# linchaobao/EPPM

Measured on AMD Instinct MI355X. Metric: Mflow-vectors/sec, higher is better.
Workload: dtype f32; 1 GPU; single 1024x436 Sintel-shape synthetic pair per step, full 3-level pyramid, patch_r=9, default defs.h parameters; 1 rank(s), independent pairs; inputs: RGBA planes resident in HBM before the timed region; outputs: interleaved float2 flow left in HBM (the PCIe-inclusive window of the reference API -- host RGB in, host u/v out -- is `host_boundary`, with --full); inputs=device-resident RGBA, outputs=device-resident float2 flow, pairs_in_flight_per_gpu=24, pairs_per_launch=8, contexts_in_flight=3, width=1024, height=436

## Files before the change

eppm_amd/_lib.py:

```python
import ctypes as C
import os

from .build import lib_path


class EppmError(RuntimeError):
    pass


class CParams(C.Structure):
    _fields_ = [("patch_r", C.c_int), ("num_iter", C.c_int), ("search_range", C.c_int), ("num_guess", C.c_int),
                ("seg_len", C.c_int), ("wmf_iters", C.c_int), ("seed", C.c_ulonglong), ("propagation", C.c_int),
                ("levels", C.c_int)]


class CTrackParams(C.Structure):
    _fields_ = [("spacing", C.c_int), ("min_eig", C.c_int64), ("fb_alpha", C.c_float), ("fb_beta", C.c_float), ("mb_alpha", C.c_float),
                ("mb_beta", C.c_float), ("capacity", C.c_int)]


class CTFilterParams(C.Structure):
    _fields_ = [("thresh", C.c_float), ("n_max", C.c_int)]


# ... 42 lines not shown
    "eppm_device_synchronize", "eppm_device_mem_info", "eppm_device_pci_bus_id", "eppm_bind_thread_to_device", "eppm_release_cached_memory", "eppm_set_launcher_stream", "eppm_set_launcher_params", "eppm_launcher_status",
    "baoCudaPatchMatchMultiscalePrepare", "baoCudaCensusTransform", "baoCudaPatchMatch", "baoCudaLeftRightCheck",
    "baoCudaOutlierRemoval", "baoCudaWeightedMedianFilter", "baoCudaFillHole", "baoCudaNNF2Flow", "baoCudaBLF_C2F",
    "baoCudaBLFCostFilterRefine", "baoCudaFlowSmoothing", "eppm_flow_to_color", "eppm_compute_color",
    "eppm_pm_rng_create", "eppm_pm_rng_reset", "eppm_pm_rng_destroy", "eppm_pm_rng_block_states", "eppm_pm_gen_rand_field",
    "eppm_pm_cost_field", "eppm_pm_seg_propagate", "eppm_pm_jump_propagate", "eppm_pm_parallel_propagate", "eppm_pm_random_search", "eppm_gauss_filter_rgba", "eppm_resize_rgba",
    "eppm_resize_flow",
    "eppm_host_register", "eppm_host_unregister", "eppm_host_is_registered", "eppm_host_alloc", "eppm_host_free",
    "eppm_compute_begin_into", "eppm_batch_compute_begin_into",
    "eppm_load_ppm", "eppm_ppm_size", "eppm_save_flo", "eppm_load_flo", "eppm_flo_size", "eppm_flow_error",
    "eppm_flow_error_border", "eppm_flow_error_percentage", "eppm_flow_cutoff", "eppm_flow_to_color_host",
    "eppm_compute_bidirectional", "eppm_compute_bidirectional_device", "eppm_batch_compute_bidirectional", "eppm_set_occlusion_params",
    "eppm_fb_occlusion", "eppm_fb_occlusion_host",
    "eppm_interpolate", "eppm_interpolate_device", "eppm_batch_interpolate", "eppm_interpolate_frames", "eppm_interpolate_host",
    "eppm_track_default_params", "eppm_track_capacity", "eppm_tracker_create", "eppm_tracker_destroy", "eppm_track_step",
    "eppm_track_step_frames", "eppm_tracker_get", "eppm_tracker_get_ended", "eppm_tracker_set", "eppm_track_step_host", "eppm_track_seeds_host",
    "eppm_push_image", "eppm_push_image_device", "eppm_set_temporal", "eppm_temporal_reset", "eppm_temporal_valid", "eppm_temporal_prior_host",
    "eppm_temporal_prior",
    "eppm_batch_set_temporal", "eppm_batch_push_images", "eppm_batch_push_images_device", "eppm_batch_temporal_valid", "eppm_batch_temporal_reset",
    "eppm_temporal_prior_batch",
    "eppm_set_stop_level", "eppm_stop_level", "eppm_flow_upsample",
    "eppm_tfilter_default_params", "eppm_tfilter_create", "eppm_tfilter_create_size", "eppm_tfilter_destroy", "eppm_tfilter_reset", "eppm_tfilter_step",
    "eppm_tfilter_step_frames", "eppm_tfilter_get", "eppm_tfilter_get_device", "eppm_tfilter_get_state", "eppm_tfilter_set_state",
    "eppm_tfilter_seed_host", "eppm_tfilter_step_host",
    "eppm_stab_default_params", "eppm_stab_create", "eppm_stab_create_size", "eppm_stab_destroy", "eppm_stab_reset", "eppm_stab_step",
    "eppm_stab_step_frames", "eppm_stab_get", "eppm_stab_get_device", "eppm_stab_get_mask", "eppm_stab_get_model", "eppm_stab_get_path",
    "eppm_stab_set_path", "eppm_gmotion_fit_host", "eppm_stab_update_host", "eppm_stab_warp_host",
    "eppm_cutdet_default_params", "eppm_cutdet_create", "eppm_cutdet_create_size", "eppm_cutdet_destroy", "eppm_cutdet_step",
    "eppm_cutdet_step_frames", "eppm_cutdet_get", "eppm_cutdet_cuts", "eppm_cutdet_host",
]


TEST_SYMBOLS = ["eppm_test_set_option", "eppm_probe_c2f_window", "eppm_probe_dispatch", "eppm_probe_fast_exp", "eppm_probe_div_const", "eppm_probe_delta_table",
                "eppm_probe_unpack_texel", "eppm_probe_pm_parity", "eppm_probe_ctx_rng_states"]

_variant = None


def select_library(variant):
    global _variant
    if _lib is not None and variant != _variant:
        raise EppmError("select_library: a library is loaded already")
    _variant = variant


def lib():
    global _lib
    if _lib is None:
        path = lib_path(_variant)
        if not os.path.exists(path):
            raise EppmError(f"{path} is missing: run eppm_amd.build() (hipcc --offload-arch=gfx950); there is no CPU fallback")
        L = C.CDLL(path)
        L.eppm_last_error.restype = C.c_char_p
        L.eppm_version.restype = C.c_char_p
        _lib = L
    return _lib


def check(status, what=""):
    if status != 0:
        raise EppmError(f"{what}: status {status}: {lib().eppm_last_error().decode()}")


def check_launcher(what=""):
    check(lib().eppm_launcher_status(), what)


def probe_dispatch(stage, *args, nout=1):
    a = (C.c_int * len(args))(*[int(v) for v in args])
    out = (C.c_int * nout)()
    check(lib().eppm_probe_dispatch(stage.encode(), a, len(args), out, nout), f"eppm_probe_dispatch {stage}")
    return tuple(out)
```

eppm_amd/csrc/c2f_device.cuh:

```cuda
#pragma once
#include "eppm_device.cuh"

#ifndef EPPM_C2F_UNROLL
#define EPPM_C2F_UNROLL 2
#endif
#ifndef EPPM_C2F_WAVES
#define EPPM_C2F_WAVES 4
#endif
#ifndef EPPM_C2F_WAVES_MIN
#define EPPM_C2F_WAVES_MIN 2
#endif
#define EPPM_C2F_OCC __attribute__((amdgpu_waves_per_eu(EPPM_C2F_WAVES_MIN, EPPM_C2F_WAVES)))
#ifndef EPPM_C2F_WIN_H
#ifdef EPPM_TOL
#define EPPM_C2F_WIN_H 50
#else
#define EPPM_C2F_WIN_H 48
#endif
#endif
#ifndef EPPM_C2F_PASS2
#define EPPM_C2F_PASS2 1
#endif
#ifndef EPPM_C2F_WIN_WAVES
#define EPPM_C2F_WIN_WAVES 4
// ... 31 lines not shown
    return pk[idx];
}

__device__ __forceinline__ bool c2f_unknown(float fvx, float fvy) { return fvx > kUnknownFlowThresh || fvy > kUnknownFlowThresh; }
__device__ __forceinline__ int c2f_centre(float f, int x) { return (int)(int16_t)(f2short(f) + x); }
__device__ __forceinline__ void c2f_store_flow(float* flow, int idx, int fx, int fy)
{
    flow[idx * 2] = (float)fx;
    flow[idx * 2 + 1] = (float)fy;
}
__device__ __forceinline__ float c2f_min(float a, float b) { return (a < b) ? a : b; }
__device__ __forceinline__ float c2f_min4(float c1, float c2, float c3, float c4) { return c2f_min(c1, c2f_min(c2, c2f_min(c3, c4))); }
template <class F>
__device__ __forceinline__ void c2f_select_best(float* flow, int x, int y, int ccx, int ccy, int w, int h, F cost_of)
{
    int bx = ccx, by = ccy;
    float min_cost = 999999;
#pragma unroll
    for (int m = 0; m < 3; m++) {
        const int cx = (int)(int16_t)(ccx + m - 1);
        if (cx < 0 || cx >= w) continue;
#pragma unroll
        for (int n = 0; n < 3; n++) {
            const int cy = (int)(int16_t)(ccy + n - 1);
            if (cy < 0 || cy >= h) continue;
            const float cv = cost_of(m, n);
            if (cv < min_cost) { min_cost = cv; bx = cx; by = cy; }
        }
    }
    flow[(y * w + x) * 2] = (float)(bx - x);
    flow[(y * w + x) * 2 + 1] = (float)(by - y);
}

template <int SPLIT>
__device__ __forceinline__ bool c2f_tile_origin(const Planes& P, int& x0, int& y0, int& part)
{
    const int tiles_x = (P.w + kBlock - 1) / kBlock, tiles = tiles_x * ((P.h + kBlock - 1) / kBlock);
    const int per_xcd = (tiles + 7) / 8;
    const int slot = SPLIT ? (blockIdx.x >> 3) / SPLIT : (blockIdx.x >> 3);
    part = SPLIT ? (blockIdx.x >> 3) % SPLIT : -1;
    const int tile = (blockIdx.x & 7) * per_xcd + slot;
    if (slot >= per_xcd || tile >= tiles) return false;
    x0 = (tile % tiles_x) * kBlock; y0 = (tile / tiles_x) * kBlock;
    return true;
}

template <int R> struct C2fSrcTile { static constexpr int TWU = kBlock + 2 * R, TW = (TWU + 15) / 16 * 16; };
struct C2fOff { int dx16, up; };

template <int R>
struct C2fTables {
    static constexpr int S = R + 1;
    C2fOff off[3][S * S];
    int rowdy[3][S];
};

constexpr int cfloor(float v) { const int t = (int)v; return ((float)t > v) ? t - 1 : t; }
template <int R>
constexpr C2fTables<R> make_c2f_tables()
{
    constexpr int S = R + 1;
    constexpr float kc[3][4] = {
        {0.177f, -0.011f, -0.003f, 0.301f},
        {0.125f, -0.357f, 0.009f, 0.308f},
        {0.205f, 0.370f, 0.011f, 0.296f},
    };
    C2fTables<R> T{};
    for (int p = 0; p < 3; p++)
        for (int ii = 0; ii < S; ii++) {
            const int i = 2 * ii - R;
            int dy[S] = {};
            int lo = 1 << 30;
            for (int jj = 0; jj < S; jj++) {
                const int j = 2 * jj - R;
                const float fx = (float)(j)*kc[p][0] + (float)(i)*kc[p][1];
// ... 159 lines not shown
```

eppm_amd/csrc/context.h:

```cpp
#pragma once

#include <algorithm>

#include "api_internal.h"

struct StageEv { const char* name; hipEvent_t a, b; };

struct eppm_ctx {
    int device = 0;
    hipStream_t stream = nullptr;
    bool own_stream = false;
    int opt_sweep_spec = -1, opt_no_split = 0;
    eppm_params prm;
    int h = 0, w = 0, nl = 0;
    int stop_level = 0;
    int npairs = 1, n_active = 1;
    char* slab = nullptr;
    size_t stride = 0;
    int H[eppm::kMaxLevels], W[eppm::kMaxLevels];
    size_t ipitch[eppm::kMaxLevels], cpitch[eppm::kMaxLevels];
    uint32_t *raw1 = nullptr, *raw2 = nullptr;
    size_t raw_pitch = 0;
    uint32_t *img1[eppm::kMaxLevels] = {}, *img2[eppm::kMaxLevels] = {}, *tmpu[eppm::kMaxLevels] = {};
    uint8_t *cen1[eppm::kMaxLevels] = {}, *cen2[eppm::kMaxLevels] = {};
    void *pk1[eppm::kMaxLevels] = {}, *pk2[eppm::kMaxLevels] = {};
    uint32_t *pc1[eppm::kMaxLevels] = {}, *pc2[eppm::kMaxLevels] = {};
    uint32_t *pp1 = nullptr, *pp2 = nullptr;
    int pp_pitch = 0, pp_pad = 0;
    int16_t *nnf1 = nullptr, *nnf2 = nullptr, *nnf_tmp = nullptr, *nnf_tmp2 = nullptr;
    float *cost1 = nullptr, *cost2 = nullptr;
    float *spec1 = nullptr, *spec2 = nullptr;
    int32_t *scand1 = nullptr, *scand2 = nullptr;
    uint32_t *wl1 = nullptr, *wl2 = nullptr;
    int16_t *seed1 = nullptr, *seed2 = nullptr;
    uint32_t* wmf_ws = nullptr;
    bool flow_pending = false;
    float *flow[eppm::kMaxLevels] = {}, *flow_tmp[eppm::kMaxLevels] = {};
    float* c2f_cost9[eppm::kMaxLevels] = {};
    float *lut_pm = nullptr, *lut_wmf = nullptr, *lut_blf = nullptr;
    eppm_pm_rng* rng = nullptr;
    float* d_uv = nullptr;
    uint32_t* d_color = nullptr;
    uint32_t* h_color = nullptr;
    uint8_t* d_rgb = nullptr;
    size_t slab_bytes = 0, h_rgb_bytes = 0, h_flow_bytes = 0;
    uint8_t* h_rgb[2] = {nullptr, nullptr};
    hipEvent_t ev_rgb[2] = {nullptr, nullptr};
    hipEvent_t ev_h2d = nullptr;
    int rgb_cur = 0;
    float* h_flow = nullptr;
    std::vector<float*> out_u, out_v;
    eppm::HostHold out_hold;
    bool have_images = false, have_flow = false;
    char* bwd = nullptr;
    size_t bwd_stride = 0, bwd_bytes = 0, h_bwd_bytes = 0;
    float* bflow[eppm::kMaxLevels] = {};
    float* d_buv = nullptr;
    uint8_t *occ1 = nullptr, *occ2 = nullptr;
    uint8_t* h_bwd = nullptr;
    float occ_alpha = 0.01f, occ_beta = 0.5f;
    bool have_bwd = false;
    bool bwd_images = false;
    char* itp = nullptr;
    size_t itp_bytes = 0, itp_plane = 0, h_itp_bytes = 0;
    uint64_t* itp_keys = nullptr;
    int32_t *itp_fill1 = nullptr, *itp_fill2 = nullptr;
    uint8_t* itp_rgb = nullptr;
    uint8_t* h_itp = nullptr;
    bool temporal = false;
    std::vector<uint8_t> tmp_snap;
    std::vector<uint8_t> tmp_valid;
    std::vector<uint8_t> tmp_seeded;
    std::vector<uint8_t> tmp_cut;
    char* tmp = nullptr;
    size_t tmp_bytes = 0, tmp_stride = 0;
    int16_t *prev_fwd = nullptr, *prev_bwd = nullptr, *prior1 = nullptr, *prior2 = nullptr, *nnf_init1 = nullptr, *nnf_init2 = nullptr;
    float *cost_init1 = nullptr, *cost_init2 = nullptr;
    int32_t* tmp_keys = nullptr;
    void tmp_drop() { std::fill(tmp_valid.begin(), tmp_valid.end(), 0); std::fill(tmp_snap.begin(), tmp_snap.end(), 0); std::fill(tmp_cut.begin(), tmp_cut.end(), 0); }
    int timing = 0;
    std::vector<StageEv> ev;
    std::vector<StageEv> ev_prep;
    std::vector<hipEvent_t> ev_pool;
    eppm::Batch bt() const { return eppm::Batch{n_active, stride}; }
    template <class T> T* of_pair(T* p, int k) const { return (T*)((char*)p + (size_t)k * stride); }
    template <class T> T* of_bwd_pair(T* p, int k) const { return (T*)((char*)p + (size_t)k * bwd_stride); }
// ... 85 lines not shown
```

eppm_amd/csrc/ctx_compute.cpp:

```cpp
#include "context.h"
#include "temporal.h"

using namespace eppm;

static int tmp_alloc(eppm_ctx* c)
{
    if (c->tmp) return EPPM_OK;
    const int L = c->nl - 1;
    const size_t n2 = (size_t)c->W[L] * c->H[L];
    Carve cv;
    for (int16_t** p : {&c->prev_fwd, &c->prev_bwd, &c->prior1, &c->prior2, &c->nnf_init1, &c->nnf_init2}) cv.plane(p, n2 * 4);
    for (float** p : {&c->cost_init1, &c->cost_init2}) cv.plane(p, n2 * 4);
    cv.plane(&c->tmp_keys, n2 * 4 * 2);
    c->tmp_stride = cv.off;
    CHK(cv.alloc(&c->tmp, &c->tmp_bytes, c->tmp_stride * c->npairs, c->device, "temporal planes"));
    for (int k = 0; k < c->npairs; k++) launch_temporal_keys_init((int32_t*)((char*)c->tmp_keys + (size_t)k * c->tmp_stride), (int)(2 * n2), c->stream);
    HIPCHK(hipGetLastError());
    return EPPM_OK;
}

static int set_temporal(eppm_ctx* c, int on)
{
    c->temporal = on != 0;
    if (!on) c->tmp_drop();
// ... 68 lines not shown
static int branch_c2f(eppm_ctx* c, Branch& d, int (*keep)(eppm_ctx*, int, float*))
{
    hipStream_t s = c->stream;
    const Batch bt = c->bt();
    const int L = c->nl - 1;
    auto blf = [&](float* dst, const float* src, int l) { launch_flow_blf(dst, src, d.guide[l], (int)(c->ipitch[l] / 4), c->W[l], c->H[l], c->W[l], c->lut_blf, s, bt); };
    const int stop = c->stop_level;
    float* r = d.a[L];
    for (int l = L - 1; l >= 0; l--) {
        if (l < stop) {
            stage_begin(c, c->ev, level_stage.s[kStageJbu][d.bwd][l]);
            float* out = (r == d.b[l]) ? d.a[l] : d.b[l];
            launch_flow_jbu(out, r, d.guide[l], (int)(c->ipitch[l] / 4), c->W[l], c->H[l], c->W[l + 1], c->H[l + 1], c->lut_blf, s, bt);
            r = out;
            CHK(keep(c, l, r));
            stage_end(c, c->ev);
            continue;
        }
        stage_begin(c, c->ev, level_stage.s[kStageUp][d.bwd][l]);
        launch_resize_flow(d.a[l], c->H[l], c->W[l], r, c->H[l + 1], c->W[l + 1], 2.0f, 2.0f, s, bt);
        stage_end(c, c->ev);
        stage_begin(c, c->ev, level_stage.s[kStageRefine][d.bwd][l], d.dominant);
        launch_c2f_refine(planes(c, l, d.swap), d.a[l], c->lut_pm, c->prm.patch_r, c->c2f_cost9[l], s, bt, c->opt_no_split != 0);
        stage_end(c, c->ev, d.dominant);
        stage_begin(c, c->ev, level_stage.s[kStageBlf][d.bwd][l]);
        blf(d.b[l], d.a[l], l);
        r = d.b[l];
        if (l > 0) CHK(keep(c, l, r));
        stage_end(c, c->ev);
    }
    if (stop > 0) return EPPM_OK;
    stage_begin(c, c->ev, d.bwd ? "flow_blf_bwd_final" : "flow_blf_final");
    float* out = (r == d.b[0]) ? d.a[0] : d.b[0];
    blf(out, r, 0);
    CHK(keep(c, 0, out));
    stage_end(c, c->ev);
    return EPPM_OK;
}

static int keep_fwd(eppm_ctx* c, int l, float* r)
{
    if (r != c->flow[l]) std::swap(c->flow[l], c->flow_tmp[l]);
    return EPPM_OK;
}

static int compute_all(eppm_ctx* c)
{
    if (!c->have_images) return set_err(EPPM_ERR_STATE, "eppm_compute: no images set");
    HIPCHK(hipSetDevice(c->device));
    c->have_bwd = false;
    hipStream_t s = c->stream;
    const Batch bt = c->bt();
    const int L = c->nl - 1, lw = c->W[L], lh = c->H[L];

    const bool tmode = c->temporal;
    bool seeded = false;
    std::fill(c->tmp_seeded.begin(), c->tmp_seeded.end(), 0);
    if (tmode) {
        CHK(tmp_alloc(c));
        TemporalArgs a{};
        for (int k = 0; k < bt.n; k++)
            if (c->tmp_valid[k]) { a.armed[k >> 5] |= 1u << (k & 31); seeded = true; }
        if (seeded) {
            a.prev[0] = c->prev_fwd; a.prior[0] = c->prior1; a.keys[0] = c->tmp_keys; a.step[0] = 1;
            a.prev[1] = c->prev_bwd; a.prior[1] = c->prior2; a.keys[1] = c->tmp_keys + (size_t)lw * lh; a.step[1] = -1;
            a.w = lw; a.h = lh; a.ndir = 2; a.nslots = bt.n; a.stride = c->tmp_stride;
            stage_begin(c, c->ev, "temporal_advect");
// ... 70 lines not shown
        HIPCHK(hipMemcpyAsync(c->of_bwd_pair(c->bflow[l], k), c->of_pair(src, k), bytes, hipMemcpyDeviceToDevice, c->stream));
    return EPPM_OK;
}

static int backward_all(eppm_ctx* c)
{
    const int L = c->nl - 1;
    Branch d{c->nnf2, c->nnf_tmp2, c->cost2, c->img2, true, true, false, nullptr};
    for (int l = 0; l <= L; l++) { d.a[l] = c->flow_tmp[l]; d.b[l] = c->d_uv; }
    stage_begin(c, c->ev, "l2_post_bwd");
    branch_nnf2flow(c, d);
    if (L > 0) CHK(keep_bwd(c, L, d.a[L]));
    stage_end(c, c->ev);
    CHK(branch_c2f(c, d, keep_bwd));

    stage_begin(c, c->ev, "fb_occlusion");
    launch_fb_occlusion(c->occ1, c->occ2, c->flow[0], c->stride, c->bflow[0], c->bwd_stride, c->h, c->w, c->occ_alpha, c->occ_beta, c->n_active, 2, c->stream);
    stage_end(c, c->ev);
    HIPCHK(hipGetLastError());
    c->have_bwd = true;
    c->bwd_images = true;
    return EPPM_OK;
}

static int compute_bidir_all(eppm_ctx* c)
{
    if (!c->have_images) return set_err(EPPM_ERR_STATE, "eppm_compute_bidirectional: no images set");
    HIPCHK(hipSetDevice(c->device));
    CHK(bwd_alloc(c));
    CHK(compute_all(c));
    return backward_all(c);
}

extern "C" int eppm_compute_device(eppm_ctx* c, void* d_flow)
{
    if (!c) return set_err(EPPM_ERR_ARG, "NULL ctx");
    CHK(compute_all(c));
    if (d_flow) HIPCHK(hipMemcpyAsync(d_flow, c->flow[0], (size_t)c->h * c->w * 8, hipMemcpyDeviceToDevice, c->stream));
    return EPPM_OK;
}

extern "C" int eppm_batch_compute_device(eppm_ctx* c, void* const* d_flows)
{
    if (!c) return set_err(EPPM_ERR_ARG, "NULL ctx");
    CHK(compute_all(c));
    if (d_flows)
        for (int k = 0; k < c->n_active; k++)
            if (d_flows[k]) HIPCHK(hipMemcpyAsync(d_flows[k], c->of_pair(c->flow[0], k), (size_t)c->h * c->w * 8, hipMemcpyDeviceToDevice, c->stream));
    return EPPM_OK;
}

static int compute_begin_impl(eppm_ctx* c, int n_out, float* const* u, float* const* v, bool bidir)
{
    CHK(bidir ? compute_bidir_all(c) : compute_all(c));
    const size_t n = (size_t)c->h * c->w;
    launch_split_flow(c->d_uv, c->flow[0], (int)n, c->stream, c->bt());
    if (bidir) {
        launch_split_flow(c->d_buv, c->bflow[0], (int)n, c->stream, Batch{c->n_active, c->bwd_stride});
        HIPCHK(pinned_lazy(&c->h_bwd, &c->h_bwd_bytes, n * 10 * c->npairs, c->device));
        for (int k = 0; k < c->n_active; k++)
            HIPCHK(hipMemcpyAsync(c->h_bwd + (size_t)k * n * 10, c->of_bwd_pair(c->d_buv, k), n * 10, hipMemcpyDeviceToHost, c->stream));
    }
    for (int k = 0; k < c->n_active; k++) {
        float* du = (u && k < n_out) ? u[k] : nullptr;
        float* dv = (v && k < n_out) ? v[k] : nullptr;
        const float* src = c->of_pair(c->d_uv, k);
        if (du && dv && c->out_hold.add2(du, dv, n * 4)) {
            HIPCHK(hipMemcpyAsync(du, src, n * 4, hipMemcpyDeviceToHost, c->stream));
            HIPCHK(hipMemcpyAsync(dv, src + n, n * 4, hipMemcpyDeviceToHost, c->stream));
            c->out_u[k] = du; c->out_v[k] = dv;
            continue;
        }
        HIPCHK(pinned_lazy(&c->h_flow, &c->h_flow_bytes, n * 8 * c->npairs, c->device));
        HIPCHK(hipMemcpyAsync(c->h_flow + (size_t)k * n * 2, src, n * 8, hipMemcpyDeviceToHost, c->stream));
        c->out_u[k] = c->out_v[k] = nullptr;
    }
    c->flow_pending = true;
    return EPPM_OK;
}
static int compute_begin(eppm_ctx* c, int n_out, float* const* u, float* const* v, bool bidir = false)
{
    const int r = compute_begin_impl(c, n_out, u, v, bidir);
// ... 138 lines not shown
```

eppm_amd/csrc/eppm_internal.h:

```cpp
#pragma once

#include <hip/hip_runtime.h>
#include <stddef.h>
#include <stdint.h>

#include "../../include/eppm.h"

namespace eppm {

constexpr int kMaxLevels = 8;
constexpr int kNumLevels = 3;
constexpr int kBlock = 16;
constexpr int kMaxS = 32;
constexpr int kWmfRadius = 4;
constexpr int kBlfRadius = 10;
constexpr int kDeltaSlots = 800;

struct Batch {
    int n;
    size_t stride;
};
constexpr Batch kOnePair = {1, 0};

#define EPPM_DECISION __attribute__((visibility("hidden")))
// ... 88 lines not shown

constexpr int kTemporalMaxSlots = 4096;
struct TemporalArgs {
    const int16_t* prev[2];
    int16_t* prior[2];
    int32_t* keys[2];
    int step[2];
    int w, h, ndir;
    int nslots;
    size_t stride;
    uint32_t armed[kTemporalMaxSlots / 32];
};
void launch_temporal_keys_init(int32_t* keys, int n, hipStream_t s);
void launch_temporal_splat(const TemporalArgs& a, hipStream_t s);
void launch_temporal_gather(const TemporalArgs& a, hipStream_t s);
void launch_temporal_snapshot(int16_t* prev, size_t prev_stride, const int16_t* nnf, int nnf_pitch, int w, int h, hipStream_t s, Batch bt = kOnePair);
void launch_nnf2flow_snapshot(float* flow, int flow_pitch, int16_t* prev, size_t prev_stride, const int16_t* nnf, int nnf_pitch, int w, int h,
                              hipStream_t s, Batch bt = kOnePair);

void launch_lr_check(int16_t* nnf1, float* cost1, const int16_t* nnf2, int w, int h, int cost_pitch, int nnf_pitch, hipStream_t s, Batch bt = kOnePair);
void launch_outlier(int16_t* nnf_out, float* cost, const int16_t* nnf_in, int w, int h, int cost_pitch, int nnf_pitch, hipStream_t s, Batch bt = kOnePair);
size_t wmf_workspace_words(int w, int h, int num_iter);
int16_t* launch_wmf(int16_t* buf_a, int16_t* buf_b, const uint32_t* img, int ipitch, int w, int h, int nnf_pitch,
                    const float* wmf_lut, int num_iter, int only_occlusion, uint32_t* ws, hipStream_t s, Batch bt = kOnePair);
void launch_fill_holes(int16_t* nnf_out, const int16_t* nnf_in, const uint32_t* img, int ipitch, int w, int h, int nnf_pitch,
                       hipStream_t s, Batch bt = kOnePair);
void launch_nnf2flow(float* flow, int flow_pitch, const int16_t* nnf, int nnf_pitch, int w, int h, hipStream_t s, Batch bt = kOnePair);

void launch_resize_flow(float* out, int outH, int outW, const float* in, int h, int w, float ratio, float post_scale, hipStream_t s, Batch bt = kOnePair);
void launch_mul_scalar(float* flow, float scale, int h, int w, hipStream_t s);
EPPM_DECISION int c2f_refine_split_factor(int w, int h, int R, int npairs = 1, bool no_split = false);
bool c2f_refine_wants_split(int w, int h, int R, int npairs = 1, bool no_split = false);
bool c2f_window_span(int R, int* span_x, int* span_y);
void launch_c2f_refine(const PlanesH& P, float* flow, const float* lut, int R, float* cost9, hipStream_t s, Batch bt = kOnePair, bool no_split = false);
void launch_flow_blf(float* out, const float* in, const uint32_t* img, int ipitch, int w, int h, int flow_pitch,
                     const float* blf_lut, hipStream_t s, Batch bt = kOnePair);
EPPM_DECISION int flow_blf_pixels_per_lane(int w, int h, int npairs = 1);
void launch_flow_jbu(float* out, const float* in_coarse, const uint32_t* img, int ipitch, int w, int h, int wc, int hc, const float* blf_lut,
                     hipStream_t s, Batch bt = kOnePair);

void launch_split_flow(float* uv, const float* flow, int n, hipStream_t s, Batch bt = kOnePair);

void launch_fb_occlusion(uint8_t* occ1, uint8_t* occ2, const float* fwd, size_t fwd_stride, const float* bwd, size_t bwd_stride, int h, int w,
                         float alpha, float beta, int npairs, int ndir, hipStream_t s);

constexpr int kInterpChunk = 4;
struct InterpArgs {
    const uint8_t* img1;
    const uint8_t* img2;
    size_t img_pitch, img_stride;
    const float* flow;
    size_t flow_stride;
    const uint8_t* occ1;
    const uint8_t* occ2;
    size_t occ_stride;
    uint64_t* keys;
    int32_t* fill1;
    int32_t* fill2;
    size_t plane;
    uint8_t* rgb;
    uint8_t* rgba[kInterpChunk];
    size_t rgba_pitch;
    int h, w, nt;
    float t[kInterpChunk];
};
void launch_interp_splat(const InterpArgs& a, int npairs, hipStream_t s);
void launch_interp_fill(const InterpArgs& a, int npairs, hipStream_t s);
void launch_interp_blend(const InterpArgs& a, int npairs, hipStream_t s);

// ... 104 lines not shown
```

eppm_amd/csrc/k_c2f_refine.hip:

```cpp
#include <type_traits>

#include "c2f_device.cuh"
#include "eppm_internal.h"

namespace eppm {

__constant__ C2fTables<9> c2f_tab9 = make_c2f_tables<9>();
__constant__ C2fTables<17> c2f_tab17 = make_c2f_tables<17>();
template <> __device__ __forceinline__ const C2fTables<9>& c2f_tables<9>() { return c2f_tab9; }
template <> __device__ __forceinline__ const C2fTables<17>& c2f_tables<17>() { return c2f_tab17; }

__global__ __launch_bounds__(256) void k_c2f_refine(PlanesH Ph, float* __restrict__ flow_, const float* __restrict__ lut, int R, size_t pstride)
{
    __shared__ EPPM_LUT_ALIGN PatchLut L;
    load_patch_lut(L, lut, R, threadIdx.y * kBlock + threadIdx.x, 256);
    __syncthreads();
    const Planes P = to_dev(Ph, pstride, blockIdx.z);
    float* __restrict__ flow = pair_ptr(flow_, pstride, blockIdx.z);
    const int x = blockIdx.x * kBlock + threadIdx.x, y = blockIdx.y * kBlock + threadIdx.y;
    if (x >= P.w || y >= P.h) return;
    const float fvx = flow[(y * P.w + x) * 2], fvy = flow[(y * P.w + x) * 2 + 1];
    if (c2f_unknown(fvx, fvy)) { c2f_store_flow(flow, y * P.w + x, 0, 0); return; }
    const int ccx = c2f_centre(fvx, x), ccy = c2f_centre(fvy, y);
    int bx = ccx, by = ccy;
// ... 323 lines not shown
    flow[(y * P.w + x) * 2 + 1] = (float)(by - y);
}

template <int SPLIT>
__global__ __launch_bounds__(256) void k_c2f_select(float* __restrict__ flow_, const float* __restrict__ cost9_, int w, int h, size_t pstride)
{
    float* __restrict__ flow = pair_ptr(flow_, pstride, blockIdx.z);
    const float* __restrict__ cost9 = pair_ptr(cost9_, pstride, blockIdx.z);
    const int x = blockIdx.x * blockDim.x + threadIdx.x, y = blockIdx.y * blockDim.y + threadIdx.y;
    if (x >= w || y >= h) return;
    const float fvx = flow[(y * w + x) * 2], fvy = flow[(y * w + x) * 2 + 1];
    if (c2f_unknown(fvx, fvy)) { c2f_store_flow(flow, y * w + x, 0, 0); return; }
    c2f_select_best(flow, x, y, c2f_centre(fvx, x), c2f_centre(fvy, y), w, h, [=](int m, int n) {
        const float* __restrict__ pc = cost9 + (size_t)(y * w + x) * 36 + m * 3 + n;
        float cv = pc[0];
        if (SPLIT == 4) {
            cv = pc[27];
            cv = c2f_min(pc[18], cv);
            cv = c2f_min(pc[9], cv);
            cv = c2f_min(pc[0], cv);
        }
        return cv;
    });
}

bool c2f_window_span(int R, int* span_x, int* span_y)
{
    if (!(R == 9 || R == 17)) return false;
    *span_x = (R == 9) ? C2fWinShape<9>::SPAN_X : C2fWinShape<17>::SPAN_X;
    *span_y = (R == 9) ? C2fWinShape<9>::SPAN_Y : C2fWinShape<17>::SPAN_Y;
    return true;
}

static bool c2f_table_ok(int w, int h, int R) { return (w + R < 32764) && (h + R < 32764); }

int c2f_refine_split_factor(int w, int h, int R, int npairs, bool no_split)
{
    if (no_split || !(R == 9 || R == 17) || !c2f_table_ok(w, h, R)) return 0;
    const int tiles = ((w + kBlock - 1) / kBlock) * ((h + kBlock - 1) / kBlock);
    if (!(tiles * npairs * 4 < EPPM_C2F_SPLIT_BELOW_WAVES)) return 0;
    auto imbalance = [&](int f) { const int wgs = tiles * f * npairs; return (float)((wgs + 255) / 256) * 256.0f / (float)wgs; };
    return (imbalance(4) < imbalance(3)) ? 4 : 3;
}
bool c2f_refine_wants_split(int w, int h, int R, int npairs, bool no_split) { return c2f_refine_split_factor(w, h, R, npairs, no_split) != 0; }

template <class F>
static void with_radius(int R, F&& f)
{
    if (R == 9) f(std::integral_constant<int, 9>{});
    else f(std::integral_constant<int, 17>{});
}

void launch_c2f_refine(const PlanesH& P, float* flow, const float* lut, int R, float* cost9, hipStream_t s, Batch bt, bool no_split)
{
    dim3 grid((P.w + kBlock - 1) / kBlock, (P.h + kBlock - 1) / kBlock, bt.n), block(kBlock, kBlock);
    const int per_xcd = (grid.x * grid.y + 7) / 8;
    dim3 grid1(per_xcd * 8, bt.n);
    if (const int f = cost9 ? c2f_refine_split_factor(P.w, P.h, R, bt.n, no_split) : 0) {
        dim3 gridf(per_xcd * f * 8, bt.n), gs((P.w + 63) / 64, (P.h + 3) / 4, bt.n), bs(64, 4);
        with_radius(R, [&](auto r) {
            if (f == 3) hipLaunchKernelGGL((k_c2f_refine_tiled<r(), 3>), gridf, block, 0, s, P, flow, lut, cost9, bt.stride);
            else hipLaunchKernelGGL((k_c2f_refine_tiled<r(), 4>), gridf, block, 0, s, P, flow, lut, cost9, bt.stride);
        });
        if (f == 3) hipLaunchKernelGGL(k_c2f_select<3>, gs, bs, 0, s, flow, cost9, P.w, P.h, bt.stride);
        else hipLaunchKernelGGL(k_c2f_select<4>, gs, bs, 0, s, flow, cost9, P.w, P.h, bt.stride);
        return;
    }
    if (!(R == 9 || R == 17) || !c2f_table_ok(P.w, P.h, R)) {
        hipLaunchKernelGGL(k_c2f_refine, grid, block, 0, s, P, flow, lut, R, bt.stride);
        return;
    }
    const bool window = (R == 9) ? EPPM_C2F_WINDOW : EPPM_C2F_WINDOW17;
    if (!window) with_radius(R, [&](auto r) { hipLaunchKernelGGL((k_c2f_refine_tiled<r(), 0>), grid1, block, 0, s, P, flow, lut, (float*)nullptr, bt.stride); });
    else if (R == 9) hipLaunchKernelGGL((k_c2f_refine_win<9>), grid1, dim3(kBlock, kBlock, 2), 0, s, P, flow, lut, bt.stride);
    else hipLaunchKernelGGL((k_c2f_refine_win4<17>), grid1, dim3(kBlock, kBlock, 4), 0, s, P, flow, lut, bt.stride);
}

}
```

eppm_amd/csrc/k_flow_blf.hip:

```cpp
#include <type_traits>

#include "eppm_device.cuh"
#include "eppm_internal.h"

#ifndef EPPM_BLF_UNROLL
#define EPPM_BLF_UNROLL 21
#endif
#ifndef EPPM_BLF_MIX
#define EPPM_BLF_MIX 3
#endif
#ifndef EPPM_BLF_MIX1
#define EPPM_BLF_MIX1 2
#endif
#ifdef EPPM_BLF_WAVES
#define EPPM_BLF_OCC __attribute__((amdgpu_waves_per_eu(EPPM_BLF_WAVES, EPPM_BLF_WAVES)))
#else
#define EPPM_BLF_OCC
#endif
#define EPPM_BLF_PRAGMA_(x) _Pragma(#x)
#define EPPM_BLF_UNROLL_PRAGMA(n) EPPM_BLF_PRAGMA_(unroll n)

namespace eppm {

constexpr int BT_W = 32, BR = kBlfRadius, BTW = BT_W + 2 * BR;
template <int PPL>
__device__ __forceinline__ constexpr bool blf_by_formula(int dx, int pixel)
{
    constexpr int M = (PPL == 1) ? EPPM_BLF_MIX1 : EPPM_BLF_MIX;
    return M == 1 ? (PPL == 2 ? pixel == 1 : (dx & 1)) : M >= 2 ? dx % M == 0 : false;
}
template <int PPL>
__global__ __launch_bounds__(256) EPPM_BLF_OCC void k_flow_blf(float* __restrict__ out_, const float* __restrict__ in_,
                                                  const uint32_t* __restrict__ img_, int ipitch, int w, int h, int fpitch,
                                                  const float* __restrict__ blf_lut, size_t pstride)
{
    float* __restrict__ out = pair_ptr(out_, pstride, blockIdx.z);
    const float* __restrict__ in = pair_ptr(in_, pstride, blockIdx.z);
    const uint32_t* __restrict__ img = pair_ptr(img_, pstride, blockIdx.z);
    constexpr int BT_H = 8 * PPL, BTH = BT_H + 2 * BR;
    __shared__ float4 s_t[BTH * BTW];
    __shared__ float s_fy[BTH * BTW];
    __shared__ float s_lut[BR + 1];
    __shared__ DeltaTab s_D;
    const int x0 = blockIdx.x * BT_W, y0 = blockIdx.y * BT_H;
    const int tid = threadIdx.y * BT_W + threadIdx.x;
    if (tid <= BR) s_lut[tid] = blf_lut[tid];
    load_delta_tab<false>(s_D, blf_lut + BR + 1, tid, 256);
    for (int t = tid; t < BTW * BTH; t += 256) {
        const int cy = y0 + t / BTW - BR, cx = x0 + t % BTW - BR;
        float4 e = make_float4(100.0f, 0.0f, 0.0f, 0.0f);
        float fy = 0.0f;
        if (cx >= 0 && cy >= 0 && cx < w && cy < h) {
            e.w = in[(cy * fpitch + cx) * 2];
            fy = in[(cy * fpitch + cx) * 2 + 1];
            if (!(e.w > kUnknownFlowThresh || fy > kUnknownFlowThresh)) {
                const rgbf c = unpack_rgb(img[cy * ipitch + cx]);
                e.x = c.x; e.y = c.y; e.z = c.z;
            }
        }
        s_t[t] = e;
        s_fy[t] = fy;
    }
    __syncthreads();
    const int x = x0 + threadIdx.x, ya = y0 + PPL * threadIdx.y;
    if (x >= w || ya >= h) return;
    const bool has_b = (PPL == 2) && (ya + 1 < h);
    const rgbf ca = unpack_rgb(img[ya * ipitch + x]);
    const rgbf cb = unpack_rgb(img[(has_b ? ya + 1 : ya) * ipitch + x]);
    float nxa = 0.f, nya = 0.f, wa = 0.f, nxb = 0.f, nyb = 0.f, wb = 0.f;
// ... 15 lines not shown
                const float coef_s = gx * gya;
                const float wgt = coef_r * coef_s;
                nxa += wgt * tp.w;
                nya += wgt * tfy;
                wa += wgt;
            }
            if (use_b) {
                const bool tab_b = EPPM_DELTA_BLF && !blf_by_formula<PPL>(dx, 1);
                const float delta_r = tab_b ? __builtin_amdgcn_fmed3f(max_abs_diff(cb, pix), 0.0f, 1.0f) : max_abs_diff(cb, pix);
                const float coef_r = tab_b ? delta_lookup_off(s_D, delta_r) : fast_exp(div_wmf2(-(delta_r * delta_r)));
                const float coef_s = gx * gyb;
                const float wgt = coef_r * coef_s;
                nxb += wgt * tp.w;
                nyb += wgt * tfy;
                wb += wgt;
            }
        }
    };
    if (PPL == 2) {
        tap_row(0, std::true_type{}, std::false_type{});
#pragma unroll 1
        for (int r = 1; r <= 2 * BR; r++) tap_row(r, std::true_type{}, std::true_type{});
        tap_row(2 * BR + 1, std::false_type{}, std::true_type{});
    } else {
#pragma unroll 1
        for (int r = 0; r <= 2 * BR; r++) tap_row(r, std::true_type{}, std::false_type{});
    }
    {
        const int ci = base + BR * BTW + BR;
        float ox = s_t[ci].w, oy = s_fy[ci];
        if (wa != 0) { ox = nxa / wa; oy = nya / wa; }
        out[(ya * fpitch + x) * 2] = ox;
        out[(ya * fpitch + x) * 2 + 1] = oy;
    }
    if (has_b) {
        const int ci = base + (BR + 1) * BTW + BR;
        float ox = s_t[ci].w, oy = s_fy[ci];
        if (wb != 0) { ox = nxb / wb; oy = nyb / wb; }
        out[((ya + 1) * fpitch + x) * 2] = ox;
        out[((ya + 1) * fpitch + x) * 2 + 1] = oy;
    }
}
int flow_blf_pixels_per_lane(int w, int h, int npairs)
{
    const int wgs2 = ((w + BT_W - 1) / BT_W) * ((h + 15) / 16) * npairs;
    return wgs2 >= 8 * 256 ? 2 : 1;
}
void launch_flow_blf(float* out, const float* in, const uint32_t* img, int ipitch, int w, int h, int flow_pitch,
                     const float* blf_lut, hipStream_t s, Batch bt)
{
    dim3 block(BT_W, 8);
    if (flow_blf_pixels_per_lane(w, h, bt.n) == 2) {
        hipLaunchKernelGGL(k_flow_blf<2>, dim3((w + BT_W - 1) / BT_W, (h + 15) / 16, bt.n), block, 0, s, out, in, img, ipitch, w, h, flow_pitch, blf_lut, bt.stride);
    } else {
        hipLaunchKernelGGL(k_flow_blf<1>, dim3((w + BT_W - 1) / BT_W, (h + 7) / 8, bt.n), block, 0, s, out, in, img, ipitch, w, h, flow_pitch, blf_lut, bt.stride);
    }
}

}
```

eppm_amd/csrc/k_pm_search.hip:

```cpp
#include "pm_device.cuh"

namespace eppm {

__device__ __forceinline__ void xorwow_skip(Xorwow& st, const uint32_t* __restrict__ skip_mat, uint32_t skip_weyl)
{
    const uint32_t v[5] = {st.v0, st.v1, st.v2, st.v3, st.v4};
    uint32_t a0 = 0, a1 = 0, a2 = 0, a3 = 0, a4 = 0;
#pragma unroll
    for (int wd = 0; wd < 5; wd++) {
        const uint32_t vw = v[wd];
#pragma unroll 8
        for (int b = 0; b < 32; b++) {
            const uint32_t* row = skip_mat + (wd * 32 + b) * 5;
            const uint32_t m = 0u - ((vw >> b) & 1u);
            a0 ^= m & row[0]; a1 ^= m & row[1]; a2 ^= m & row[2]; a3 ^= m & row[3]; a4 ^= m & row[4];
        }
    }
    st.v0 = a0; st.v1 = a1; st.v2 = a2; st.v3 = a3; st.v4 = a4;
    st.d += skip_weyl;
}

__global__ __launch_bounds__(64) void k_pm_rand_table(PmRngDev rng, uint32_t* __restrict__ work, int16_t* __restrict__ tab, int G)
{
    const int block_id = blockIdx.x, lane = threadIdx.x;
    const size_t so = ((size_t)block_id * 64 + lane) * 6;
    Xorwow st = load_state(work + so);
    int16_t* __restrict__ out = tab + (size_t)block_id * 512 * G + rng.per_lane * lane;
    for (int q = 0; q < rng.per_lane; q++) out[q] = (int16_t)xorwow_next(st);
    xorwow_skip(st, rng.skip_mat, rng.skip_weyl);
    store_state(work + so, st);
}
void launch_pm_rand_table(const PmRngDev& rng, uint32_t* work, int16_t* tab, int G, hipStream_t s)
{
    hipLaunchKernelGGL(k_pm_rand_table, dim3(rng.gx * rng.gy), dim3(64), 0, s, rng, work, tab, G);
}

template <int RT, int PK = 0, bool TAB = false, int ROWS = 4>
__global__ __launch_bounds__(576) EPPM_SEARCH_OCC void k_pm_random_search(PmBatch B, PmRngDev rng, const float* __restrict__ lut, int R,
                                                          int search_range, int G)
{
    static_assert(ROWS == 4 || (ROWS == 2 && TAB && RT != 0), "eighth-block workgroups read their numbers from the table");
    using LUT = typename SearchLut<RT>::type;
    constexpr int PIXW = 16 * ROWS, NSUB = kBlock / ROWS;
    constexpr int TW = (RT == 0) ? 1 : kBlock + 2 * RT, TH = (RT == 0) ? 1 : ROWS + 2 * RT;
    __shared__ float4 s_src[TW * TH];
    __shared__ EPPM_LUT_ALIGN LUT L;
    __shared__ int16_t s_rand[TAB ? 2 : 8 * 512];
    __shared__ float s_cost[8][64];
    __shared__ int s_guess[8][64];
    __shared__ uint32_t s_state[TAB ? 2 : 64 * 6];
    const unsigned nprob = B.n * B.npairs, bq = blockIdx.x % nprob, brest = blockIdx.x / nprob;
    const int bxx = brest % rng.gx, byy = brest / rng.gx;
    const PmProblem pr = pm_problem(B, bq);
    const int tid = threadIdx.x;
    const int tile_y = byy / NSUB, quarter = byy % NSUB;
    const int block_id = tile_y * rng.gx + bxx;
    load_patch_lut(L, lut, R, tid, blockDim.x);
    if (!TAB && tid < 64) {
        const size_t so = ((size_t)block_id * 64 + tid) * 6;
        Xorwow st = load_state(pr.rng_work + so);
        const int base = rng.per_lane * tid;
        for (int q = 0; q < rng.per_lane; q++) s_rand[base + q] = (int16_t)xorwow_next(st);
        if (quarter == 0) store_state(s_state + tid * 6, st);
    }
    const Planes P = to_dev(pr.P);
    if (RT != 0) {
        const int x0 = bxx * kBlock - RT, y0 = tile_y * kBlock + quarter * ROWS - RT;
        for (int t = tid; t < TW * TH; t += blockDim.x) {
            const int sy = iclamp(y0 + t / TW, 0, P.h - 1), sx = iclamp(x0 + t % TW, 0, P.w - 1);
            s_src[t] = P.pk1[(unsigned)(sy * P.pitch + sx)];
        }
    }
    __syncthreads();
    const int lane = tid % PIXW, k = tid / PIXW;
    if (!TAB && k == G) {
        if (quarter == 0) {
            const size_t so = ((size_t)block_id * 64 + lane) * 6;
            Xorwow st = load_state(s_state + lane * 6);
            xorwow_skip(st, rng.skip_mat, rng.skip_weyl);
            store_state(pr.rng_work_next + so, st);
        }
    }
    const int pix = quarter * PIXW + lane;
    const int x = bxx * kBlock + (pix & 15), y = tile_y * kBlock + (pix >> 4);
    const bool inimg = (k < G) && (x < P.w && y < P.h);
    const int nidx = y * B.npitch + x, cidx = y * B.cpitch + x;
    int bx = 0, by = 0;
    int mag = search_range;
    for (int q = 0; q < k; q++) if (mag / 2 >= 1) mag /= 2;
    if (inimg) { bx = pr.nnf[nidx * 2]; by = pr.nnf[nidx * 2 + 1]; }
    int gx = 0, gy = 0;
    bool evaluate = false;
    if (inimg) {
        uint32_t rdn1, rdn2;
        if (TAB) {
            const uint32_t two = *reinterpret_cast<const uint32_t*>(rng.rand_tab + ((size_t)block_id * G + k) * 512 + 2 * pix);
            rdn1 = (uint32_t)(int32_t)(int16_t)(two & 0xffffu);
            rdn2 = (uint32_t)(int32_t)(int16_t)(two >> 16);
        } else {
            rdn1 = (uint32_t)(int32_t)s_rand[512 * k + 2 * pix];
            rdn2 = (uint32_t)(int32_t)s_rand[512 * k + 2 * pix + 1];
        }
        const int xmin = max(bx - mag, 0), xmax = min(bx + mag + 1, P.w + 1);
// ... 67 lines not shown
```

eppm_amd/csrc/pm_device.cuh:

```cuda
#pragma once
#include "eppm_device.cuh"

#ifndef EPPM_PARITY_SEARCH
#define EPPM_PARITY_SEARCH 1
#endif
#ifndef EPPM_PARITY_SPEC
#define EPPM_PARITY_SPEC 0
#endif
#ifndef EPPM_PARITY_COST
#define EPPM_PARITY_COST 1
#endif
#ifndef EPPM_COST_FIELD_TILE
#define EPPM_COST_FIELD_TILE 1
#endif
#ifndef EPPM_LPC9
#ifdef EPPM_TOL
#define EPPM_LPC9 32
#else
#define EPPM_LPC9 16
#endif
#endif
#ifndef EPPM_LPC17
#define EPPM_LPC17 64
#endif
// ... 13 lines not shown
#ifndef EPPM_SWEEP_PRE
#define EPPM_SWEEP_PRE 1
#endif
#ifndef EPPM_SWEEP_GB
#define EPPM_SWEEP_GB 7
#endif
#ifndef EPPM_SWEEP_GB_SPEC
#define EPPM_SWEEP_GB_SPEC 3
#endif
#ifndef EPPM_SWEEP_TILE
#define EPPM_SWEEP_TILE 1
#endif
#ifdef EPPM_SWEEP_WAVES
#define EPPM_SWEEP_OCC __attribute__((amdgpu_waves_per_eu(EPPM_SWEEP_WAVES, EPPM_SWEEP_WAVES)))
#else
#define EPPM_SWEEP_OCC
#endif
#ifndef EPPM_SPEC_COOP17_MAX
#define EPPM_SPEC_COOP17_MAX 32
#endif
#ifndef EPPM_MERGED_COOP9_MAX
#define EPPM_MERGED_COOP9_MAX 16
#endif
#ifdef EPPM_SEARCH_WAVES
#define EPPM_SEARCH_OCC __attribute__((amdgpu_waves_per_eu(EPPM_SEARCH_WAVES, EPPM_SEARCH_WAVES)))
#else
#define EPPM_SEARCH_OCC
#endif
#ifndef EPPM_SEARCH_SKIP_SAME
#define EPPM_SEARCH_SKIP_SAME 1
#endif
#ifndef EPPM_SEARCH_HALF_BELOW_WGS
#define EPPM_SEARCH_HALF_BELOW_WGS 1024
#endif
#ifndef EPPM_SEARCH_PK17
#define EPPM_SEARCH_PK17 1
#endif

namespace eppm {

__device__ __forceinline__ Planes to_dev(const PlanesH& h)
{
    Planes p;
    p.pk1 = (const float4*)h.pk1; p.pk2 = (const float4*)h.pk2;
    p.w = h.w; p.h = h.h; p.pitch = h.pitch;
    return p;
}

__device__ __forceinline__ PmProblem pm_problem(const PmBatch& B, unsigned q)
{
    PmProblem p = B.p[q % (unsigned)B.n];
    const unsigned pair = q / (unsigned)B.n;
    p.P.pk1 = pair_ptr_opt(p.P.pk1, B.stride, pair);
    p.P.pk2 = pair_ptr_opt(p.P.pk2, B.stride, pair);
    p.P.pc1 = pair_ptr_opt(p.P.pc1, B.stride, pair);
    p.P.pc2 = pair_ptr_opt(p.P.pc2, B.stride, pair);
    p.P.pp1 = pair_ptr_opt(p.P.pp1, B.stride, pair);
    p.P.pp2 = pair_ptr_opt(p.P.pp2, B.stride, pair);
    p.cost = pair_ptr_opt(p.cost, B.stride, pair);
    p.nnf = pair_ptr_opt(p.nnf, B.stride, pair);
    p.nnf_alt = pair_ptr_opt(p.nnf_alt, B.stride, pair);
    p.spec = pair_ptr_opt(p.spec, B.stride, pair);
    p.scand = pair_ptr_opt(p.scand, B.stride, pair);
    p.wl = pair_ptr_opt(p.wl, B.stride, pair);
    p.seed = pair_ptr_opt(p.seed, B.stride, pair);
    p.rng_work = pair_ptr_opt(p.rng_work, B.stride, pair);
// ... 210 lines not shown
```

Baseline: 229.9 Mflow-vectors/s.

## Balance c2f tiles across XCDs, fuse output write into BLF, pad search tile

Three unrelated changes land together. The c2f refine tile-to-XCD mapping now spreads the full tiles and the ragged bottom-row tiles evenly over the eight XCDs instead of handing out contiguous chunks. The final flow bilateral filter can also write straight into the caller's device output buffers, which removes the trailing device-to-device copy for each pair. The radius-9 random-search shared-memory tile row stride is padded to a multiple of 16 float4, meant to avoid LDS bank conflicts, at the cost of slightly more LDS per workgroup.

Result: no change. 230.8 Mflow-vectors/s, median of 6 (+0.4%).

```diff
diff --git a/eppm_amd/_lib.py b/eppm_amd/_lib.py
--- a/eppm_amd/_lib.py
+++ b/eppm_amd/_lib.py
@@ -98,7 +98,7 @@
 
 
 TEST_SYMBOLS = ["eppm_test_set_option", "eppm_probe_c2f_window", "eppm_probe_dispatch", "eppm_probe_fast_exp", "eppm_probe_div_const", "eppm_probe_delta_table",
-                "eppm_probe_unpack_texel", "eppm_probe_pm_parity", "eppm_probe_ctx_rng_states"]
+                "eppm_probe_unpack_texel", "eppm_probe_pm_parity", "eppm_probe_ctx_rng_states", "eppm_probe_c2f_tile_order"]
 
 _variant = None
 
@@ -137,3 +137,11 @@
     out = (C.c_int * nout)()
     check(lib().eppm_probe_dispatch(stage.encode(), a, len(args), out, nout), f"eppm_probe_dispatch {stage}")
     return tuple(out)
+
+
+def probe_c2f_tile_order(w, h, split=0):
+    n = C.c_int(0)
+    check(lib().eppm_probe_c2f_tile_order(int(w), int(h), int(split), None, None, 0, C.byref(n)), "eppm_probe_c2f_tile_order")
+    tile, part = (C.c_int * n.value)(), (C.c_int * n.value)()
+    check(lib().eppm_probe_c2f_tile_order(int(w), int(h), int(split), tile, part, n.value, C.byref(n)), "eppm_probe_c2f_tile_order")
+    return list(tile), list(part)
diff --git a/eppm_amd/csrc/c2f_device.cuh b/eppm_amd/csrc/c2f_device.cuh
--- a/eppm_amd/csrc/c2f_device.cuh
+++ b/eppm_amd/csrc/c2f_device.cuh
@@ -87,15 +87,38 @@
     flow[(y * w + x) * 2 + 1] = (float)(by - y);
 }
 
+#ifndef EPPM_C2F_XCD_BALANCE
+#define EPPM_C2F_XCD_BALANCE 1
+#endif
+__host__ __device__ inline int c2f_slots_per_xcd(int w, int h)
+{
+    const int tiles_x = (w + kBlock - 1) / kBlock, tiles_y = (h + kBlock - 1) / kBlock;
+    if (!EPPM_C2F_XCD_BALANCE) return (tiles_x * tiles_y + 7) / 8;
+    const int ragged = (h % kBlock) ? tiles_x : 0, full = tiles_x * tiles_y - ragged;
+    return (full + 7) / 8 + (ragged + 7) / 8;
+}
+__host__ __device__ inline int c2f_tile_of_slot(int bx, int w, int h, int split, int& part)
+{
+    const int tiles_x = (w + kBlock - 1) / kBlock, tiles = tiles_x * ((h + kBlock - 1) / kBlock);
+    const int xcd = bx & 7, slot = split ? (bx >> 3) / split : (bx >> 3);
+    part = split ? (bx >> 3) % split : -1;
+    if (!EPPM_C2F_XCD_BALANCE) {
+        const int per_xcd = (tiles + 7) / 8, tile = xcd * per_xcd + slot;
+        return (slot >= per_xcd || tile >= tiles) ? -1 : tile;
+    }
+    const int ragged = (h % kBlock) ? tiles_x : 0, full = tiles - ragged;
+    const int f0 = (xcd * full) >> 3, f1 = ((xcd + 1) * full) >> 3;
+    const int r0 = (xcd * ragged) >> 3, r1 = ((xcd + 1) * ragged) >> 3;
+    if (slot < f1 - f0) return f0 + slot;
+    const int rs = slot - (f1 - f0);
+    return (rs < r1 - r0) ? full + r0 + rs : -1;
+}
 template <int SPLIT>
 __device__ __forceinline__ bool c2f_tile_origin(const Planes& P, int& x0, int& y0, int& part)
 {
-    const int tiles_x = (P.w + kBlock - 1) / kBlock, tiles = tiles_x * ((P.h + kBlock - 1) / kBlock);
-    const int per_xcd = (tiles + 7) / 8;
-    const int slot = SPLIT ? (blockIdx.x >> 3) / SPLIT : (blockIdx.x >> 3);
-    part = SPLIT ? (blockIdx.x >> 3) % SPLIT : -1;
-    const int tile = (blockIdx.x & 7) * per_xcd + slot;
-    if (slot >= per_xcd || tile >= tiles) return false;
+    const int tiles_x = (P.w + kBlock - 1) / kBlock;
+    const int tile = c2f_tile_of_slot(blockIdx.x, P.w, P.h, SPLIT, part);
+    if (tile < 0) return false;
     x0 = (tile % tiles_x) * kBlock; y0 = (tile / tiles_x) * kBlock;
     return true;
 }
diff --git a/eppm_amd/csrc/context.h b/eppm_amd/csrc/context.h
--- a/eppm_amd/csrc/context.h
+++ b/eppm_amd/csrc/context.h
@@ -52,6 +52,8 @@
     std::vector<float*> out_u, out_v;
     eppm::HostHold out_hold;
     bool have_images = false, have_flow = false;
+    const eppm::BlfOut2* out2 = nullptr;
+    bool out2_done = false;
     char* bwd = nullptr;
     size_t bwd_stride = 0, bwd_bytes = 0, h_bwd_bytes = 0;
     float* bflow[eppm::kMaxLevels] = {};
diff --git a/eppm_amd/csrc/ctx_compute.cpp b/eppm_amd/csrc/ctx_compute.cpp
--- a/eppm_amd/csrc/ctx_compute.cpp
+++ b/eppm_amd/csrc/ctx_compute.cpp
@@ -124,7 +124,9 @@
     if (stop > 0) return EPPM_OK;
     stage_begin(c, c->ev, d.bwd ? "flow_blf_bwd_final" : "flow_blf_final");
     float* out = (r == d.b[0]) ? d.a[0] : d.b[0];
-    blf(out, r, 0);
+    const BlfOut2* o2 = d.bwd ? nullptr : c->out2;
+    launch_flow_blf(out, r, d.guide[0], (int)(c->ipitch[0] / 4), c->W[0], c->H[0], c->W[0], c->lut_blf, s, bt, o2);
+    if (o2) c->out2_done = true;
     CHK(keep(c, 0, out));
     stage_end(c, c->ev);
     return EPPM_OK;
@@ -261,22 +263,36 @@
     return backward_all(c);
 }
 
+#ifndef EPPM_BLF_OUT2
+#define EPPM_BLF_OUT2 1
+#endif
+static int compute_device(eppm_ctx* c, void* const* d_flows, int n)
+{
+    BlfOut2 o2 = {};
+    bool any = false;
+    if (EPPM_BLF_OUT2 && d_flows && c->n_active <= kBlfOut2Max)
+        for (int k = 0; k < n && k < c->n_active; k++) { o2.p[k] = (float*)d_flows[k]; any = any || d_flows[k]; }
+    c->out2 = any ? &o2 : nullptr;
+    c->out2_done = false;
+    const int r = compute_all(c);
+    c->out2 = nullptr;
+    CHK(r);
+    if (d_flows && !c->out2_done)
+        for (int k = 0; k < n && k < c->n_active; k++)
+            if (d_flows[k]) HIPCHK(hipMemcpyAsync(d_flows[k], c->of_pair(c->flow[0], k), (size_t)c->h * c->w * 8, hipMemcpyDeviceToDevice, c->stream));
+    return EPPM_OK;
+}
+
 extern "C" int eppm_compute_device(eppm_ctx* c, void* d_flow)
 {
     if (!c) return set_err(EPPM_ERR_ARG, "NULL ctx");
-    CHK(compute_all(c));
-    if (d_flow) HIPCHK(hipMemcpyAsync(d_flow, c->flow[0], (size_t)c->h * c->w * 8, hipMemcpyDeviceToDevice, c->stream));
-    return EPPM_OK;
+    return compute_device(c, d_flow ? &d_flow : nullptr, 1);
 }
 
 extern "C" int eppm_batch_compute_device(eppm_ctx* c, void* const* d_flows)
 {
     if (!c) return set_err(EPPM_ERR_ARG, "NULL ctx");
-    CHK(compute_all(c));
-    if (d_flows)
-        for (int k = 0; k < c->n_active; k++)
-            if (d_flows[k]) HIPCHK(hipMemcpyAsync(d_flows[k], c->of_pair(c->flow[0], k), (size_t)c->h * c->w * 8, hipMemcpyDeviceToDevice, c->stream));
-    return EPPM_OK;
+    return compute_device(c, d_flows, c->n_active);
 }
 
 static int compute_begin_impl(eppm_ctx* c, int n_out, float* const* u, float* const* v, bool bidir)
diff --git a/eppm_amd/csrc/eppm_internal.h b/eppm_amd/csrc/eppm_internal.h
--- a/eppm_amd/csrc/eppm_internal.h
+++ b/eppm_amd/csrc/eppm_internal.h
@@ -144,9 +144,13 @@
 EPPM_DECISION int c2f_refine_split_factor(int w, int h, int R, int npairs = 1, bool no_split = false);
 bool c2f_refine_wants_split(int w, int h, int R, int npairs = 1, bool no_split = false);
 bool c2f_window_span(int R, int* span_x, int* span_y);
+EPPM_DECISION int c2f_refine_slots(int w, int h, int split);
+EPPM_DECISION int c2f_refine_tile_of_slot(int slot, int w, int h, int split, int* part);
 void launch_c2f_refine(const PlanesH& P, float* flow, const float* lut, int R, float* cost9, hipStream_t s, Batch bt = kOnePair, bool no_split = false);
+constexpr int kBlfOut2Max = 32;
+struct BlfOut2 { float* p[kBlfOut2Max]; };
 void launch_flow_blf(float* out, const float* in, const uint32_t* img, int ipitch, int w, int h, int flow_pitch,
-                     const float* blf_lut, hipStream_t s, Batch bt = kOnePair);
+                     const float* blf_lut, hipStream_t s, Batch bt = kOnePair, const BlfOut2* out2 = nullptr);
 EPPM_DECISION int flow_blf_pixels_per_lane(int w, int h, int npairs = 1);
 void launch_flow_jbu(float* out, const float* in_coarse, const uint32_t* img, int ipitch, int w, int h, int wc, int hc, const float* blf_lut,
                      hipStream_t s, Batch bt = kOnePair);
diff --git a/eppm_amd/csrc/k_c2f_refine.hip b/eppm_amd/csrc/k_c2f_refine.hip
--- a/eppm_amd/csrc/k_c2f_refine.hip
+++ b/eppm_amd/csrc/k_c2f_refine.hip
@@ -379,6 +379,9 @@
     return true;
 }
 
+int c2f_refine_slots(int w, int h, int split) { return c2f_slots_per_xcd(w, h) * 8 * (split ? split : 1); }
+int c2f_refine_tile_of_slot(int slot, int w, int h, int split, int* part) { return c2f_tile_of_slot(slot, w, h, split, *part); }
+
 static bool c2f_table_ok(int w, int h, int R) { return (w + R < 32764) && (h + R < 32764); }
 
 int c2f_refine_split_factor(int w, int h, int R, int npairs, bool no_split)
@@ -401,7 +404,7 @@
 void launch_c2f_refine(const PlanesH& P, float* flow, const float* lut, int R, float* cost9, hipStream_t s, Batch bt, bool no_split)
 {
     dim3 grid((P.w + kBlock - 1) / kBlock, (P.h + kBlock - 1) / kBlock, bt.n), block(kBlock, kBlock);
-    const int per_xcd = (grid.x * grid.y + 7) / 8;
+    const int per_xcd = c2f_slots_per_xcd(P.w, P.h);
     dim3 grid1(per_xcd * 8, bt.n);
     if (const int f = cost9 ? c2f_refine_split_factor(P.w, P.h, R, bt.n, no_split) : 0) {
         dim3 gridf(per_xcd * f * 8, bt.n), gs((P.w + 63) / 64, (P.h + 3) / 4, bt.n), bs(64, 4);
diff --git a/eppm_amd/csrc/k_flow_blf.hip b/eppm_amd/csrc/k_flow_blf.hip
--- a/eppm_amd/csrc/k_flow_blf.hip
+++ b/eppm_amd/csrc/k_flow_blf.hip
@@ -29,12 +29,14 @@
     constexpr int M = (PPL == 1) ? EPPM_BLF_MIX1 : EPPM_BLF_MIX;
     return M == 1 ? (PPL == 2 ? pixel == 1 : (dx & 1)) : M >= 2 ? dx % M == 0 : false;
 }
-template <int PPL>
+template <int PPL, bool OUT2>
 __global__ __launch_bounds__(256) EPPM_BLF_OCC void k_flow_blf(float* __restrict__ out_, const float* __restrict__ in_,
                                                   const uint32_t* __restrict__ img_, int ipitch, int w, int h, int fpitch,
-                                                  const float* __restrict__ blf_lut, size_t pstride)
+                                                  const float* __restrict__ blf_lut, size_t pstride, std::conditional_t<OUT2, BlfOut2, int> o2)
 {
     float* __restrict__ out = pair_ptr(out_, pstride, blockIdx.z);
+    float* __restrict__ out2 = nullptr;
+    if constexpr (OUT2) out2 = o2.p[blockIdx.z];
     const float* __restrict__ in = pair_ptr(in_, pstride, blockIdx.z);
     const uint32_t* __restrict__ img = pair_ptr(img_, pstride, blockIdx.z);
     constexpr int BT_H = 8 * PPL, BTH = BT_H + 2 * BR;
@@ -116,6 +118,7 @@
         if (wa != 0) { ox = nxa / wa; oy = nya / wa; }
         out[(ya * fpitch + x) * 2] = ox;
         out[(ya * fpitch + x) * 2 + 1] = oy;
+        if (OUT2 && out2) { out2[(ya * fpitch + x) * 2] = ox; out2[(ya * fpitch + x) * 2 + 1] = oy; }
     }
     if (has_b) {
         const int ci = base + (BR + 1) * BTW + BR;
@@ -123,6 +126,7 @@
         if (wb != 0) { ox = nxb / wb; oy = nyb / wb; }
         out[((ya + 1) * fpitch + x) * 2] = ox;
         out[((ya + 1) * fpitch + x) * 2 + 1] = oy;
+        if (OUT2 && out2) { out2[((ya + 1) * fpitch + x) * 2] = ox; out2[((ya + 1) * fpitch + x) * 2 + 1] = oy; }
     }
 }
 int flow_blf_pixels_per_lane(int w, int h, int npairs)
@@ -131,13 +135,16 @@
     return wgs2 >= 8 * 256 ? 2 : 1;
 }
 void launch_flow_blf(float* out, const float* in, const uint32_t* img, int ipitch, int w, int h, int flow_pitch,
-                     const float* blf_lut, hipStream_t s, Batch bt)
+                     const float* blf_lut, hipStream_t s, Batch bt, const BlfOut2* out2)
 {
     dim3 block(BT_W, 8);
+    const dim3 grid2((w + BT_W - 1) / BT_W, (h + 15) / 16, bt.n), grid1((w + BT_W - 1) / BT_W, (h + 7) / 8, bt.n);
     if (flow_blf_pixels_per_lane(w, h, bt.n) == 2) {
-        hipLaunchKernelGGL(k_flow_blf<2>, dim3((w + BT_W - 1) / BT_W, (h + 15) / 16, bt.n), block, 0, s, out, in, img, ipitch, w, h, flow_pitch, blf_lut, bt.stride);
+        if (out2) hipLaunchKernelGGL((k_flow_blf<2, true>), grid2, block, 0, s, out, in, img, ipitch, w, h, flow_pitch, blf_lut, bt.stride, *out2);
+        else hipLaunchKernelGGL((k_flow_blf<2, false>), grid2, block, 0, s, out, in, img, ipitch, w, h, flow_pitch, blf_lut, bt.stride, 0);
     } else {
-        hipLaunchKernelGGL(k_flow_blf<1>, dim3((w + BT_W - 1) / BT_W, (h + 7) / 8, bt.n), block, 0, s, out, in, img, ipitch, w, h, flow_pitch, blf_lut, bt.stride);
+        if (out2) hipLaunchKernelGGL((k_flow_blf<1, true>), grid1, block, 0, s, out, in, img, ipitch, w, h, flow_pitch, blf_lut, bt.stride, *out2);
+        else hipLaunchKernelGGL((k_flow_blf<1, false>), grid1, block, 0, s, out, in, img, ipitch, w, h, flow_pitch, blf_lut, bt.stride, 0);
     }
 }
 
diff --git a/eppm_amd/csrc/k_pm_search.hip b/eppm_amd/csrc/k_pm_search.hip
--- a/eppm_amd/csrc/k_pm_search.hip
+++ b/eppm_amd/csrc/k_pm_search.hip
@@ -42,7 +42,9 @@
     static_assert(ROWS == 4 || (ROWS == 2 && TAB && RT != 0), "eighth-block workgroups read their numbers from the table");
     using LUT = typename SearchLut<RT>::type;
     constexpr int PIXW = 16 * ROWS, NSUB = kBlock / ROWS;
-    constexpr int TW = (RT == 0) ? 1 : kBlock + 2 * RT, TH = (RT == 0) ? 1 : ROWS + 2 * RT;
+    constexpr int TWU = (RT == 0) ? 1 : kBlock + 2 * RT, TH = (RT == 0) ? 1 : ROWS + 2 * RT;
+    constexpr int TW = (RT == 9 && EPPM_SEARCH_TILE_PAD) ? (TWU + 15) / 16 * 16 : TWU;
+    static_assert(!(RT == 9 && EPPM_SEARCH_TILE_PAD) || (TW % 16 == 0 && TW >= TWU), "radius 9: row stride = 0 mod 256 B (conflict-free ds_read_b128)");
     __shared__ float4 s_src[TW * TH];
     __shared__ EPPM_LUT_ALIGN LUT L;
     __shared__ int16_t s_rand[TAB ? 2 : 8 * 512];
@@ -66,9 +68,10 @@
     const Planes P = to_dev(pr.P);
     if (RT != 0) {
         const int x0 = bxx * kBlock - RT, y0 = tile_y * kBlock + quarter * ROWS - RT;
-        for (int t = tid; t < TW * TH; t += blockDim.x) {
-            const int sy = iclamp(y0 + t / TW, 0, P.h - 1), sx = iclamp(x0 + t % TW, 0, P.w - 1);
-            s_src[t] = P.pk1[(unsigned)(sy * P.pitch + sx)];
+        for (int t = tid; t < TWU * TH; t += blockDim.x) {
+            const int ry = t / TWU, rx = t % TWU;
+            const int sy = iclamp(y0 + ry, 0, P.h - 1), sx = iclamp(x0 + rx, 0, P.w - 1);
+            s_src[ry * TW + rx] = P.pk1[(unsigned)(sy * P.pitch + sx)];
         }
     }
     __syncthreads();
diff --git a/eppm_amd/csrc/pm_device.cuh b/eppm_amd/csrc/pm_device.cuh
--- a/eppm_amd/csrc/pm_device.cuh
+++ b/eppm_amd/csrc/pm_device.cuh
@@ -69,6 +69,9 @@
 #endif
 #ifndef EPPM_SEARCH_HALF_BELOW_WGS
 #define EPPM_SEARCH_HALF_BELOW_WGS 1024
+#endif
+#ifndef EPPM_SEARCH_TILE_PAD
+#define EPPM_SEARCH_TILE_PAD 1
 #endif
 #ifndef EPPM_SEARCH_PK17
 #define EPPM_SEARCH_PK17 1
```
